# ai4sre/RCAEval

Measured on AMD Instinct MI355X. Metric: Fisher-z CI tests/sec + PC skeleton wall-time (2000 vars), 1/2/4/8 MI355X, higher is better.
Workload: dtype f64

## Files before the change

include/pcgpu.h:

```cpp
#ifndef PCGPU_H
#define PCGPU_H

#include <stdint.h>

#ifdef __cplusplus
extern "C" {
#endif

#define PCG_OK 0
#define PCG_ERR_INVALID -1
#define PCG_ERR_OOM -2
#define PCG_ERR_HIP -3
#define PCG_ERR_SINGULAR -4
#define PCG_ERR_DOMAIN -5
#define PCG_ERR_RCCL -6
#define PCG_ERR_OVERFLOW -7
#define PCG_ERR_PEER -8

#define PCG_FLAG_FULL_P 0x1
#define PCG_FLAG_RECORD 0x2
#define PCG_FLAG_EXACT_ALL 0x4

#define PCG_MAX_LEVELS 32
#define PCG_MAX_DEPTH 12
// ... 28 lines not shown
    int32_t s[PCG_MAX_DEPTH];
    double p;
} pcg_record;

#define PCG_ABI_VERSION 4
int pcg_abi_info(int64_t *stats_bytes, int64_t *record_bytes, int32_t *version);

int pcg_create(int device, pcg_handle **out);
int pcg_destroy(pcg_handle *h);
const char *pcg_last_error(pcg_handle *h);
int pcg_set_stream(pcg_handle *h, void *hip_stream);
int pcg_set_capacity(pcg_handle *h, int64_t record_capacity, int64_t deferred_capacity);
int pcg_set_record_sample(pcg_handle *h, int64_t modulus, int64_t residue);

#define PCG_TUNE_SMALL 0
#define PCG_TUNE_SMALL_QCAP 1
#define PCG_TUNE_LDS_DEEP 2
#define PCG_TUNE_LDS_SPILL_MIN 3
#define PCG_TUNE_WAVE_LO 4
#define PCG_TUNE_SCREEN_MASK 5
#define PCG_TUNE_NODE_BLOCKS 6
#define PCG_TUNE_EXPORT_INLINE 7
#define PCG_TUNE_NB 8
#define PCG_TUNE_NBW 9
#define PCG_TUNE_HOST_TRACE 10
#define PCG_TUNE_K1_I8 11
#define PCG_TUNE_K1_CRT 12
#define PCG_TUNE_K1_CRT_MINN 13
#define PCG_TUNE_K1_CRT_BITS 14
#define PCG_TUNE_K1_CRT_KS 15
#define PCG_TUNE_K1_I8_KS 16
#define PCG_TUNE_K1_SUPER_ORDER 17
#define PCG_TUNE_L1Z 18
#define PCG_TUNE_COUNT 19
int pcg_set_tuning(pcg_handle *h, int key, int64_t value);
int pcg_get_tuning(pcg_handle *h, int key, int64_t *value);

int pcg_corr(pcg_handle *h, const double *X, int64_t N, int64_t n, int64_t ldx,
             double *C, int64_t ldc);

int pcg_corr_shard_bytes(pcg_handle *h, int64_t n, int64_t N, int world, int64_t *bytes_per_rank);
int pcg_k1_plan_signature(pcg_handle *h, int64_t n, int64_t N, int64_t *signature);
int pcg_corr_shard_rows(int64_t n, int world, int64_t *rows_per_rank);
int pcg_corr_shard(pcg_handle *h, const double *X, int64_t N, int64_t n, int64_t ldx, int rank,
                   int world, double *packed);
int pcg_corr_shard_finish(pcg_handle *h, const double *gathered, int64_t N, int64_t n, int world,
                          double *C, int64_t ldc);

int pcg_skeleton(pcg_handle *h, const double *C, int64_t n, int64_t ldc, int64_t N,
                 double alpha, int max_depth, int flags, int8_t *removed_level,
                 pcg_stats *stats);

int pcg_pc_skeleton(pcg_handle *h, const double *X, int64_t N, int64_t n, int64_t ldx, double *C,
                    int64_t ldc, double alpha, int max_depth, int flags, int8_t *removed_level,
                    pcg_stats *stats);

int pcg_degrees(pcg_handle *h, int32_t *deg_host, int64_t capacity);

int pcg_sepset_count(pcg_handle *h, int64_t *count, int32_t *words_per_row);
int pcg_sepset_export(pcg_handle *h, int32_t *xy_host ,
                      uint64_t *bits_host , int64_t count);
int pcg_sepset_export_device(pcg_handle *h, int32_t *xy_dev, uint64_t *bits_dev, int64_t count);
int pcg_set_sepset_buffers(pcg_handle *h, int32_t *xy_dev, uint64_t *bits_dev, int64_t capacity);
int pcg_sepset_target(pcg_handle *h, int32_t *in_caller, int64_t *capacity_needed);

int pcg_record_count(pcg_handle *h, int64_t *count, int64_t *near_alpha_count);
int pcg_record_export(pcg_handle *h, pcg_record *rec_host, int64_t count,
                      pcg_record *near_host, int64_t near_count);

typedef struct {
    const double *X;
    int64_t N, n, ldx;
    double *C;
    int64_t ldc;
    int8_t *removed_level;
// ... 111 lines not shown
```

rcaeval_amd/_lib.py:

```python
from __future__ import annotations

import ctypes
import os

_HERE = os.path.dirname(os.path.abspath(__file__))
LIB_PATH = os.environ.get("PCG_LIB_PATH") or os.path.join(_HERE, "libpcgpu.so")

PCG_OK = 0
PCG_ERR_INVALID = -1
PCG_ERR_OOM = -2
PCG_ERR_HIP = -3
PCG_ERR_SINGULAR = -4
PCG_ERR_DOMAIN = -5
PCG_ERR_RCCL = -6
PCG_ERR_OVERFLOW = -7
PCG_ERR_PEER = -8

PCG_FLAG_FULL_P = 0x1
PCG_FLAG_RECORD = 0x2
PCG_FLAG_EXACT_ALL = 0x4

PCG_MAX_LEVELS = 32
PCG_ABI_VERSION = 4
PCG_RM_STATUS = 64
PCG_MAX_DEPTH = 12
PCG_MAX_LEVEL_DEPTH = 30

PCG_DRIVER_LEVELS = 0
PCG_DRIVER_SMALL = 1
PCG_DRIVER_SMALL_RERUN = 2
DRIVER_NAMES = {PCG_DRIVER_LEVELS: "levels", PCG_DRIVER_SMALL: "small", PCG_DRIVER_SMALL_RERUN: "small_rerun"}

TUNE_KEYS = {
    "SMALL": 0, "SMALL_QCAP": 1, "LDS_DEEP": 2, "LDS_SPILL_MIN": 3, "WAVE_LO": 4, "SCREEN_MASK": 5,
    "NODE_BLOCKS": 6, "EXPORT_INLINE": 7, "NB": 8, "NBW": 9, "HOST_TRACE": 10, "K1_I8": 11, "K1_CRT": 12,
    "K1_CRT_MINN": 13, "K1_CRT_BITS": 14, "K1_CRT_KS": 15, "K1_I8_KS": 16, "K1_SUPER_ORDER": 17,
    "L1Z": 18,
}

I64 = ctypes.c_int64
I32 = ctypes.c_int32
P = ctypes.c_void_p
D = ctypes.c_double


class PcgStats(ctypes.Structure):
    _fields_ = [
        ("tests", I64 * PCG_MAX_LEVELS),
        ("calls", I64 * PCG_MAX_LEVELS),
        ("indep", I64 * PCG_MAX_LEVELS),
        ("exact", I64 * PCG_MAX_LEVELS),
        ("near_alpha", I64 * PCG_MAX_LEVELS),
        ("edges_after", I64 * PCG_MAX_LEVELS),
        ("max_degree", I32 * PCG_MAX_LEVELS),
        ("level_ms", D * PCG_MAX_LEVELS),
        ("kernel_ms", D * PCG_MAX_LEVELS),
        ("levels", I32),
        ("error", I32),
        ("screened", I64 * PCG_MAX_LEVELS),
        ("driver", I32),
        ("driver_pad", I32),
    ]

    def as_dict(self) -> dict:
        L = self.levels
        return {
            "levels": L,
            "error": self.error,
            "tests": list(self.tests[:L]),
            "calls": list(self.calls[:L]),
            "indep": list(self.indep[:L]),
# ... 3 lines not shown
            "max_degree": list(self.max_degree[:L]),
            "level_ms": list(self.level_ms[:L]),
            "kernel_ms": list(self.kernel_ms[:L]),
            "screened": list(self.screened[:L]),
            "driver": DRIVER_NAMES.get(self.driver, str(self.driver)),
        }


class PcgRecord(ctypes.Structure):
    _fields_ = [("a", I32), ("b", I32), ("d", I32), ("s", I32 * PCG_MAX_DEPTH), ("p", D)]


class PcgCase(ctypes.Structure):
    _fields_ = [("X", P), ("N", I64), ("n", I64), ("ldx", I64), ("C", P), ("ldc", I64),
                ("removed_level", P), ("sep_xy", P), ("sep_bits", P)]


class PcgCaseResult(ctypes.Structure):
    _fields_ = [("rc", I32), ("rc_pad", I32), ("sep_rows", I64), ("near_alpha_count", I64),
                ("stats", PcgStats), ("deg", (I32 * 64) * PCG_MAX_LEVELS)]


SIGNATURES = [
    ("pcg_abi_info", I32, [ctypes.POINTER(I64), ctypes.POINTER(I64), ctypes.POINTER(I32)]),
    ("pcg_create", I32, [ctypes.c_int, ctypes.POINTER(P)]),
    ("pcg_destroy", I32, [P]),
    ("pcg_last_error", ctypes.c_char_p, [P]),
    ("pcg_set_stream", I32, [P, P]),
    ("pcg_set_capacity", I32, [P, I64, I64]),
    ("pcg_set_record_sample", I32, [P, I64, I64]),
    ("pcg_set_tuning", I32, [P, ctypes.c_int, I64]),
    ("pcg_get_tuning", I32, [P, ctypes.c_int, ctypes.POINTER(I64)]),
    ("pcg_k1_plan_signature", I32, [P, I64, I64, ctypes.POINTER(I64)]),
    ("pcg_corr", I32, [P, P, I64, I64, I64, P, I64]),
    ("pcg_corr_shard_rows", I32, [I64, ctypes.c_int, ctypes.POINTER(I64)]),
    ("pcg_corr_shard_bytes", I32, [P, I64, I64, ctypes.c_int, ctypes.POINTER(I64)]),
    ("pcg_corr_shard", I32, [P, P, I64, I64, I64, ctypes.c_int, ctypes.c_int, P]),
    ("pcg_corr_shard_finish", I32, [P, P, I64, I64, ctypes.c_int, P, I64]),
    ("pcg_skeleton", I32, [P, P, I64, I64, I64, D, ctypes.c_int, ctypes.c_int, P, ctypes.POINTER(PcgStats)]),
    ("pcg_pc_skeleton", I32, [P, P, I64, I64, I64, P, I64, D, ctypes.c_int, ctypes.c_int, P,
                          ctypes.POINTER(PcgStats)]),
    ("pcg_degrees", I32, [P, P, I64]),
    ("pcg_sepset_count", I32, [P, ctypes.POINTER(I64), ctypes.POINTER(I32)]),
    ("pcg_sepset_export", I32, [P, P, P, I64]),
    ("pcg_sepset_export_device", I32, [P, P, P, I64]),
    ("pcg_set_sepset_buffers", I32, [P, P, P, I64]),
    ("pcg_sepset_target", I32, [P, ctypes.POINTER(I32), ctypes.POINTER(I64)]),
    ("pcg_record_count", I32, [P, ctypes.POINTER(I64), ctypes.POINTER(I64)]),
    ("pcg_record_export", I32, [P, P, I64, P, I64]),
    ("pcg_skeleton_batch", I32, [P, ctypes.POINTER(PcgCase), I64, D, ctypes.c_int, ctypes.c_int,
                                 ctypes.POINTER(PcgCaseResult)]),
    ("pcg_batch_abi_info", I32, [ctypes.POINTER(I64), ctypes.POINTER(I64)]),
    ("pcg_batch_near_export", I32, [P, I64, P, I64]),
    ("pcg_skeleton_init", I32, [P, P, I64, I64, I64, D, ctypes.c_int, P]),
    ("pcg_level_begin", I32, [P, ctypes.c_int, ctypes.POINTER(I64), ctypes.POINTER(I32), ctypes.POINTER(P)]),
    ("pcg_level_run", I32, [P, I64, I64]),
    ("pcg_level_end", I32, [P, ctypes.POINTER(PcgStats)]),
    ("pcg_level_image_totals", I32, [P, ctypes.c_int, ctypes.POINTER(I64), ctypes.POINTER(I64)]),
    ("pcg_level_chunk_work", I32, [P, P, I64]),
    ("pcg_level_split", I32, [P, ctypes.c_int, ctypes.c_int, ctypes.POINTER(I64), ctypes.POINTER(I64)]),
    ("pcg_set_removal_buffer", I32, [P, P, I64]),
    ("pcg_level_packed_words", I32, [I64, ctypes.POINTER(I64)]),
    ("pcg_level_pack", I32, [P, P, ctypes.c_int]),
    ("pcg_level_merge", I32, [P, P, ctypes.c_int]),
    ("pcg_set_world_size", I32, [P, ctypes.c_int]),
    ("pcg_set_narrow_degree", I32, [P, ctypes.c_int]),
# ... 102 lines not shown
```

rcaeval_amd/csrc/api.hip:

```cpp
#include <hip/hip_runtime.h>

#include <algorithm>
#include <cerrno>
#include <cstdlib>
#include <cstring>

#include "handle.h"

int pcg_fail(pcg_handle *h, int code, const char *fmt, ...) {
    if (h) {
        char buf[1024];
        va_list ap;
        va_start(ap, fmt);
        vsnprintf(buf, sizeof(buf), fmt, ap);
        va_end(ap);
        h->err = buf;
    }
    return code;
}

bool pcg_ensure(pcg_handle *h, DevBuf &b, size_t bytes) {
    if (bytes == 0) bytes = 16;
    if (b.bytes >= bytes) return true;
    if (b.p) {
// ... 44 lines not shown
}

extern "C" int pcg_batch_abi_info(int64_t *case_bytes, int64_t *result_bytes) {
    if (case_bytes) *case_bytes = (int64_t)sizeof(pcg_case);
    if (result_bytes) *result_bytes = (int64_t)sizeof(pcg_case_result);
    return PCG_OK;
}

namespace {
struct TuneSpec {
    const char *env;
    int64_t dflt, lo, hi;
};
const TuneSpec kTune[PCG_TUNE_COUNT] = {
    {"PCG_SMALL", 1, 0, 1},
    {"PCG_SMALL_QCAP", 1024, 1, 1024},
    {"PCG_LDS_DEEP", 20, 12, 20},
    {"PCG_LDS_SPILL_MIN", 10000000, 0, INT64_MAX},
    {"PCG_WAVE_LO", 0, 0, PCG_MAX_LEVEL_DEPTH + 1},
    {"PCG_SCREEN_MASK", -1, -1, 0x1c},
    {"PCG_NODE_BLOCKS", 0x18, 0, 0x1c},
    {"PCG_EXPORT_INLINE", 16384, 0, INT64_MAX},
    {"PCG_NB", 0, 0, 1 << 24},
    {"PCG_NBW", 512, 1, 1 << 24},
    {"PCG_HOST_TRACE", 0, 0, 1},
    {"PCG_K1_I8", 1, 0, 1},
    {"PCG_K1_CRT", 1, 0, 1},
    {"PCG_K1_CRT_MINN", 256, 1, 1 << 24},
    {"PCG_K1_CRT_BITS", 53, 32, 63},
    {"PCG_K1_CRT_KS", 0, 0, 16},
    {"PCG_K1_I8_KS", 0, 0, 256},
    {"PCG_K1_SUPER_ORDER", 1, 0, 1},
    {"PCG_L1Z", 1, 0, 1},
};
}

void pcg_tuning_defaults(int64_t *tune) {
    for (int k = 0; k < PCG_TUNE_COUNT; ++k) {
        int64_t v = kTune[k].dflt;
        if (const char *e = getenv(kTune[k].env)) {
            char *end = nullptr;
            errno = 0;
            const long long p = strtoll(e, &end, 0);
            if (end == e || *end != '\0' || errno == ERANGE || p < kTune[k].lo || p > kTune[k].hi)
                fprintf(stderr, "pcgpu: ignoring %s=%s (not an integer in [%lld, %lld]); using %lld\n", kTune[k].env, e,
                        (long long)kTune[k].lo, (long long)kTune[k].hi, (long long)kTune[k].dflt);
            else
                v = p;
        }
        tune[k] = v;
    }
}

extern "C" int pcg_set_tuning(pcg_handle *h, int key, int64_t value) {
    if (!h || key < 0 || key >= PCG_TUNE_COUNT || value < kTune[key].lo || value > kTune[key].hi)
        return pcg_fail(h, PCG_ERR_INVALID, "pcg_set_tuning: key %d value %lld", key, (long long)value);
    h->tune[key] = value;
    return PCG_OK;
}

extern "C" int pcg_get_tuning(pcg_handle *h, int key, int64_t *value) {
    if (!h || !value || key < 0 || key >= PCG_TUNE_COUNT)
        return pcg_fail(h, PCG_ERR_INVALID, "pcg_get_tuning: key %d", key);
    *value = h->tune[key];
    return PCG_OK;
}
// ... 99 lines not shown
```

rcaeval_amd/csrc/corr.hip:

```cpp
#include <hip/hip_runtime.h>

#include <algorithm>
#include <cmath>
#include <cstring>
#include <vector>

#include "handle.h"

namespace {

typedef double d4 __attribute__((ext_vector_type(4)));

#ifndef PCG_K1_TILE
#define PCG_K1_TILE 64
#endif
#ifndef PCG_K1_XCD
#define PCG_K1_XCD 1
#endif
#ifndef PCG_K1_KS
#define PCG_K1_KS 0
#endif
constexpr int TILE = PCG_K1_TILE;
constexpr int WT = TILE / 32;
constexpr int RS = 256 / TILE;
// ... 389 lines not shown
}

constexpr int CRT_KMAX = 24;
constexpr int CRT_L = 6;
constexpr int CRT_T = 256;
constexpr int CRT_KB = 4;
#ifndef PCG_CRT_PR
#define PCG_CRT_PR 8
#endif
constexpr int CRT_PR = PCG_CRT_PR;
#ifndef PCG_CRT_KP
#define PCG_CRT_KP 1
#endif
constexpr int CRT_KP = PCG_CRT_KP;
constexpr int CRT_PL = CRT_PR - 2 * CRT_KP;
static_assert(CRT_PR * 16384 <= 160 * 1024 && CRT_PL >= CRT_KP && CRT_PL % CRT_KP == 0, "CRT LDS ring");
constexpr int CRT_MAXKB = 4095;
constexpr int CRT_UNIT = CRT_T * CRT_T;
static const int kCrtModuli[CRT_KMAX] = {256, 255, 253, 251, 247, 241, 239, 233, 229, 227, 223, 217,
                                         211, 199, 197, 193, 191, 181, 179, 173, 167, 163, 157, 151};

struct CrtTab {
    int k, b, L;
    int m[CRT_KMAX];
    int y[CRT_KMAX];
    float finv[CRT_KMAX];
    double dinv[CRT_KMAX];
    uint32_t wlo[CRT_KMAX], whi[CRT_KMAX];
    uint32_t cneg[CRT_KMAX];
    uint32_t Mi[CRT_KMAX][2 * CRT_L];
    uint32_t M[2 * CRT_L];
};

template <int L>
struct CrtAcc {
    uint32_t l[2 * L];
    float fs;
};

template <int L>
__device__ __forceinline__ void crt_acc_init(CrtAcc<L> &a) {
#pragma unroll
    for (int l = 0; l < 2 * L; ++l) a.l[l] = 0;
    a.fs = 0.0f;
}

template <int L>
__device__ __forceinline__ void crt_acc_add(CrtAcc<L> &a, uint32_t z, int mi, const CrtTab &tab) {
    a.fs = fmaf((float)z, tab.finv[mi], a.fs);
#pragma unroll
    for (int l = 0; l < 2 * L; ++l) a.l[l] = __umul24(z, tab.Mi[mi][l]) + a.l[l];
}

template <int L>
__device__ __forceinline__ double crt_value(const CrtAcc<L> &a, const CrtTab &tab, int ei, int ej) {
    const int32_t qq = (int32_t)floorf(a.fs + 0.5f);
    uint32_t lim[CRT_L];
    int32_t carry = 0;
#pragma unroll
    for (int l = 0; l < CRT_L; ++l) {
        int32_t v0 = carry, v1;
        if (l < L) v0 += (int32_t)a.l[2 * l] - qq * (int32_t)tab.M[2 * l];
        const uint32_t lo = (uint32_t)v0 & 0xffffu;
        v1 = v0 >> 16;
        if (l < L) v1 += (int32_t)a.l[2 * l + 1] - qq * (int32_t)tab.M[2 * l + 1];
        lim[l] = lo | ((uint32_t)v1 << 16);
// ... 87 lines not shown
        const int m = tab.m[mi];
        if (m == 256) {
#pragma unroll
            for (int q = 0; q < 4; ++q) pk[q] = (int)pack4(lo[4 * q], lo[4 * q + 1], lo[4 * q + 2], lo[4 * q + 3]);
        } else {
            const f2 fi = {tab.finv[mi], tab.finv[mi]};
            const f2 nm = {-(float)m, -(float)m};
            const f2 mg = {12582912.0f, 12582912.0f};
            const uint32_t wl = tab.wlo[mi], wh = tab.whi[mi], cn = tab.cneg[mi];
#pragma unroll
            for (int q = 0; q < 4; ++q) {
                uint32_t bb[4];
#pragma unroll
                for (int u = 0; u < 4; u += 2) {
                    const int i = 4 * q + u;
                    const float x0 = (float)(int)__builtin_amdgcn_udot4(
                        lo[i], wl, __builtin_amdgcn_udot4(hi[i], wh, cn, false), false);
                    const float x1 = (float)(int)__builtin_amdgcn_udot4(
                        lo[i + 1], wl, __builtin_amdgcn_udot4(hi[i + 1], wh, cn, false), false);
                    const f2 x = {x0, x1};
                    const f2 qv = __builtin_elementwise_fma(x, fi, mg) - mg;
                    const f2 rv = __builtin_elementwise_fma(qv, nm, x) + mg;
                    const float r0 = rv.x, r1 = rv.y;
                    bb[u] = __float_as_uint(r0);
                    bb[u + 1] = __float_as_uint(r1);
                }
                pk[q] = (int)pack4(bb[0], bb[1], bb[2], bb[3]);
            }
        }
        *reinterpret_cast<v4i *>(dst + mi * plane) = pk;
    }
}

__global__ __launch_bounds__(512, 1) void k_xtx_crt(const int8_t *R, int TB, int64_t plane, int T, int ntiles, int ks,
                                                  int kb, CrtTab tab, int64_t u0, int64_t nu, uint8_t *out) {
    extern __shared__ __attribute__((aligned(16))) unsigned char smem[];
    int64_t lin = blockIdx.x;
    {
        const int64_t per = gridDim.x / 8;
        lin = (blockIdx.x % 8) * per + blockIdx.x / 8;
        if (lin >= nu) return;
    }
    const int64_t u = u0 + lin;
    const int t = (int)(u % ntiles);
    const int64_t sm = u / ntiles;
    const int mi = (int)(sm / ks), slab = (int)(sm % ks);
    int bi, bj;
    tile_of(t, T, bi, bj);
    const int tb0 = slab * kb, tb1 = min(TB, tb0 + kb);
    const int tid = threadIdx.x, lane = tid & 63, w = tid >> 6;
    const int r = lane & 31, hh = lane >> 5;
    const int wr = w >> 2, wc = w & 3;

    v16i acc[4][2];
#pragma unroll
    for (int a = 0; a < 4; ++a)
#pragma unroll
        for (int b = 0; b < 2; ++b)
#pragma unroll
            for (int q = 0; q < 16; ++q) acc[a][b][q] = 0;

    const int8_t *Rm = R + (int64_t)mi * plane;
    const int8_t *srcA = Rm + (int64_t)(bi * 4 + (tid >> 7)) * TB * 2048 + (tid & 127) * 16;
    const int8_t *srcB = Rm + (int64_t)(bj * 4 + (tid >> 7)) * TB * 2048 + (tid & 127) * 16;
    const int nkb = tb1 - tb0;
    auto stage = [&](int g) {
        const int64_t tb = tb0 + min(g, nkb - 1);
        unsigned char *dst = smem + (g % CRT_PR) * 16384 + w * 1024;
        __builtin_amdgcn_global_load_lds((const __attribute__((address_space(1))) void *)(srcA + tb * 2048),
                                         (__attribute__((address_space(3))) void *)dst, 16, 0, 0);
        __builtin_amdgcn_global_load_lds((const __attribute__((address_space(1))) void *)(srcB + tb * 2048),
                                         (__attribute__((address_space(3))) void *)(dst + 8192), 16, 0, 0);
    };
    const unsigned char *fa0 = smem + (2 * wr * 2048 + hh * 1024 + r * 16);
    const unsigned char *fb0 = smem + (8192 + wc * 2048 + hh * 1024 + r * 16);
    v4i af[2][CRT_KP][4], bf[2][CRT_KP][2];
    auto frag = [&](int g, int sl) {
#pragma unroll
// ... 51 lines not shown
#pragma unroll
    for (int a = 0; a < 4; ++a)
#pragma unroll
        for (int b = 0; b < 2; ++b) {
            v4i pk = {0, 0, 0, 0};
#pragma unroll
            for (int q = 0; q < 16; ++q) {
                const int v = acc[a][b][q];
                uint32_t rr;
                if (m == 256) {
                    rr = (uint32_t)v & 255u;
                } else {
                    const int t = __mul24(v >> 16, c16) + (v & 0xffff);
                    const float tf = (float)t;
                    int x = (int)fmaf(-rintf(tf * finv), fm, tf);
                    x += x < 0 ? m : 0;
                    x -= x >= m ? m : 0;
                    rr = (uint32_t)x;
                }
                pk[q >> 2] |= (int)(rr << (8 * (q & 3)));
            }
            *reinterpret_cast<v4i *>(o + (a * 2 + b) * 1024) = pk;
        }
}

__device__ __forceinline__ int crt_unit_offset(int li, int lj) {
    const int wr = li >> 7, a = (li >> 5) & 3, rr = li & 31;
    const int hh = (rr >> 2) & 1, q = (rr & 3) | ((rr >> 3) << 2);
    const int wc = lj >> 6, b = (lj >> 5) & 1, r = lj & 31;
    return ((((wr * 4 + wc) * 4 + a) * 2 + b) * 64 + r + 32 * hh) * 16 + q;
}

template <int L>
__global__ __launch_bounds__(256) void k_crt_diag(const uint8_t *Rs, int T, int ntiles, int ks, CrtTab tab,
                                                 const int *expo, int n, double scale, double *sd) {
    const int i = blockIdx.x * blockDim.x + threadIdx.x;
    if (i >= n) return;
    const int bi = i / CRT_T;
    const int t = bi * T - bi * (bi - 1) / 2;
    const int ei = expo[i];
    if (ei == K1_NONFINITE) {
        sd[i] = NAN;
        return;
    }
    const int k = tab.k;
    const int64_t ustride = (int64_t)ntiles * CRT_UNIT;
    const uint8_t *src = Rs + (int64_t)t * CRT_UNIT + crt_unit_offset(i % CRT_T, i % CRT_T);
    uint32_t sv[CRT_KMAX];
#pragma unroll
    for (int mi = 0; mi < CRT_KMAX; ++mi) sv[mi] = 0;
    for (int s = 0; s < ks; ++s) {
        uint32_t b[CRT_KMAX];
#pragma unroll
        for (int mi = 0; mi < CRT_KMAX; ++mi) b[mi] = src[((int64_t)min(mi, k - 1) * ks + s) * ustride];
#pragma unroll
        for (int mi = 0; mi < CRT_KMAX; ++mi) sv[mi] += b[mi];
    }
    CrtAcc<L> acc;
    crt_acc_init(acc);
#pragma unroll
    for (int mi = 0; mi < CRT_KMAX; ++mi)
        if (mi < k) crt_acc_add(acc, crt_mod(__umul24(sv[mi], (uint32_t)tab.y[mi]), tab.m[mi], tab.finv[mi]), mi, tab);
    sd[i] = sqrt(crt_value(acc, tab, ei, ei) * scale);
}

template <int L>
__global__ __launch_bounds__(256) void k_crt_finish(const uint8_t *Rs, int T, int ntiles, int ks, CrtTab tab,
                                                   const int *expo, int n, const double *sd, double scale, double *C,
                                                   int64_t ldc) {
    const int64_t gid = (int64_t)blockIdx.x * blockDim.x + threadIdx.x;
    const int t = (int)(gid >> 14), rem = (int)((gid >> 2) & 4095), g = (int)(gid & 3);
    if (t >= ntiles) return;
    int bi, bj;
    tile_of(t, T, bi, bj);
    const int lane = rem & 63, wab = rem >> 6;
    const int r = lane & 31, hh = lane >> 5;
    const int b = wab & 1, a = (wab >> 1) & 3, wr = wab >> 5, wc = (wab >> 3) & 3;
    const int j = bj * CRT_T + wc * 64 + b * 32 + r;
    const int ibase = bi * CRT_T + wr * 128 + a * 32 + 4 * hh + 8 * g;
    if (j >= n || ibase > j) return;
    const int k = tab.k;
    const int ej = expo[j];
    const int64_t ustride = (int64_t)ntiles * CRT_UNIT;
    const uint8_t *src = Rs + (int64_t)t * CRT_UNIT + rem * 16 + 4 * g;
    uint32_t se[CRT_KMAX], so[CRT_KMAX];
#pragma unroll
    for (int mi = 0; mi < CRT_KMAX; ++mi) se[mi] = so[mi] = 0;
    for (int s = 0; s < ks; ++s) {
        uint32_t wd[CRT_KMAX];
#pragma unroll
        for (int mi = 0; mi < CRT_KMAX; ++mi)
            wd[mi] = *reinterpret_cast<const uint32_t *>(src + ((int64_t)min(mi, k - 1) * ks + s) * ustride);
#pragma unroll
        for (int mi = 0; mi < CRT_KMAX; ++mi) {
            se[mi] += wd[mi] & 0x00ff00ffu;
            so[mi] += (wd[mi] >> 8) & 0x00ff00ffu;
        }
    }
    CrtAcc<L> acc[4];
#pragma unroll
    for (int q4 = 0; q4 < 4; ++q4) crt_acc_init(acc[q4]);
#pragma unroll
    for (int mi = 0; mi < CRT_KMAX; ++mi) {
        if (mi >= k) continue;
        const int m = tab.m[mi];
        const float fi = tab.finv[mi];
        const uint32_t y = (uint32_t)tab.y[mi];
#pragma unroll
        for (int q4 = 0; q4 < 4; ++q4) {
            const uint32_t sv = (((q4 & 1) ? so[mi] : se[mi]) >> (16 * (q4 >> 1))) & 0xffffu;
            crt_acc_add(acc[q4], crt_mod(__umul24(sv, y), m, fi), mi, tab);
        }
    }
    const double sj = sd[j];
#pragma unroll
    for (int q4 = 0; q4 < 4; ++q4) {
        const int i = ibase + q4;
// ... 2 lines not shown
        const double gv = (ei == K1_NONFINITE || ej == K1_NONFINITE) ? NAN : crt_value(acc[q4], tab, ei, ej);
        const double si = sd[i];
        C[(int64_t)i * ldc + j] = corr_of(gv, scale, si, sj);
        if (i != j) C[(int64_t)j * ldc + i] = corr_of(gv, scale, sj, si);
    }
}

int split_k_i8(const int64_t *tune, int n, int64_t N, int *kb_out) {
    const int T = (n + 63) / 64;
    const int ntiles = T * (T + 1) / 2;
    const int TB = (int)((N + 63) / 64 * 2);
    int ks = (int)std::max<int64_t>(1, (PCG_K1_BLOCKS + ntiles / 2) / ntiles);
    if (tune[PCG_TUNE_K1_I8_KS] > 0) ks = (int)tune[PCG_TUNE_K1_I8_KS];
    ks = std::min(ks, std::max(1, TB / 2));
    ks = std::min(ks, 256);
    int kb = (TB + ks - 1) / ks;
    kb = std::min(kb, K1_I8_MAXK / K1_TB);
    *kb_out = kb;
    return (TB + kb - 1) / kb;
}

struct K1Tune {
    int64_t v[PCG_TUNE_COUNT];
    explicit K1Tune(const pcg_handle *h) {
        if (h) memcpy(v, h->tune, sizeof(v));
        else pcg_tuning_defaults(v);
    }
};

struct CrtPlan {
    CrtTab tab;
    int T = 0, ntiles = 0, ks = 0, kb = 0, TB = 0, CBp = 0;
    int64_t units = 0;
};

static void big_mul_small(uint32_t *x, int L, uint32_t m) {
    uint64_t c = 0;
    for (int l = 0; l < L; ++l) {
        const uint64_t v = (uint64_t)x[l] * m + c;
        x[l] = (uint32_t)v;
        c = v >> 32;
    }
}
static uint32_t big_div_small(const uint32_t *x, int L, uint32_t m, uint32_t *q) {
    uint64_t r = 0;
    for (int l = L - 1; l >= 0; --l) {
        const uint64_t v = (r << 32) | x[l];
        q[l] = (uint32_t)(v / m);
        r = v % m;
    }
    return (uint32_t)r;
}

static bool crt_plan_build(const int64_t *tune, int n, int64_t N, CrtPlan &p);

bool crt_plan(const int64_t *tune, int n, int64_t N, CrtPlan &p) {
    struct Entry {
        int64_t key[7];
        bool ok;
        CrtPlan plan;
    };
    thread_local Entry e{{-1, -1, -1, -1, -1, -1, -1}, false, CrtPlan{}};
    const int64_t key[7] = {n, N, tune[PCG_TUNE_K1_I8], tune[PCG_TUNE_K1_CRT], tune[PCG_TUNE_K1_CRT_MINN],
                            tune[PCG_TUNE_K1_CRT_BITS], tune[PCG_TUNE_K1_CRT_KS]};
    if (memcmp(key, e.key, sizeof(key)) != 0) {
        e.ok = crt_plan_build(tune, n, N, e.plan);
        memcpy(e.key, key, sizeof(key));
    }
    if (e.ok) p = e.plan;
    return e.ok;
}

static bool crt_plan_build(const int64_t *tune, int n, int64_t N, CrtPlan &p) {
    if (!tune[PCG_TUNE_K1_I8] || !tune[PCG_TUNE_K1_CRT] || n < tune[PCG_TUNE_K1_CRT_MINN]) return false;
    const int bmin = (int)std::min<int64_t>(63, std::max<int64_t>(32, tune[PCG_TUNE_K1_CRT_BITS]));
    double lm = 0.0;
    int k = 0, b = 0;
    for (; k < CRT_KMAX; ++k) {
        lm += std::log2((double)kCrtModuli[k]);
        b = (int)std::floor((lm - std::log2((double)N) - 1.0 - 0.01) / 2.0);
        if (b >= bmin) { ++k; break; }
    }
    if (b < bmin) return false;
    b = std::min(b, 63);
    CrtTab &t = p.tab;
    memset(&t, 0, sizeof(t));
    t.k = k;
    t.b = b;
    uint32_t M[CRT_L] = {1, 0, 0, 0, 0, 0};
    for (int i = 0; i < k; ++i) big_mul_small(M, CRT_L, (uint32_t)kCrtModuli[i]);
    t.L = (int)std::floor(lm / 32.0) + 1;
    if (lm > 32.0 * t.L - 1.0) ++t.L;
    if (t.L > CRT_L) return false;
    for (int l = 0; l < CRT_L; ++l) {
        t.M[2 * l] = M[l] & 0xffffu;
        t.M[2 * l + 1] = M[l] >> 16;
    }
    for (int i = 0; i < k; ++i) {
        const uint32_t m = (uint32_t)kCrtModuli[i];
        t.m[i] = (int)m;
        t.finv[i] = 1.0f / (float)m;
        t.dinv[i] = 1.0 / (double)m;
        uint32_t Mi32[CRT_L], mq[CRT_L];
        big_div_small(M, CRT_L, m, Mi32);
        for (int l = 0; l < CRT_L; ++l) {
            t.Mi[i][2 * l] = Mi32[l] & 0xffffu;
// ... 15 lines not shown
        t.whi[i] = wh;
        uint64_t pb = 1;
        for (int s2 = 0; s2 < b; ++s2) pb = (pb * 2) % m;
        t.cneg[i] = 0u - (uint32_t)pb;
    }
    p.T = (n + CRT_T - 1) / CRT_T;
    p.ntiles = p.T * (p.T + 1) / 2;
    p.CBp = p.T * 4;
    p.TB = (int)((N + 63) / 64 * 2);
    int best = 1;
    double best_cost = 1e300;
    const int force = (int)tune[PCG_TUNE_K1_CRT_KS];
    for (int ks = 1; ks <= 16; ++ks) {
        int kbk = (p.TB + ks - 1) / ks;
        kbk = (kbk + CRT_KB - 1) / CRT_KB * CRT_KB;
        const int kse = (p.TB + kbk - 1) / kbk;
        if (kse != ks || kbk > CRT_MAXKB) continue;
        const int64_t U = (int64_t)p.ntiles * k * ks;
        const double cost = force > 0 ? (double)std::abs(ks - force)
                                      : (double)((U + 255) / 256) * kbk * 0.3 + (double)U * 0.026;
        if (cost < best_cost) {
            best_cost = cost;
            best = ks;
        }
    }
    {
        int kbk = (p.TB + best - 1) / best;
        kbk = (kbk + CRT_KB - 1) / CRT_KB * CRT_KB;
        if (kbk > CRT_MAXKB) return false;
        p.kb = kbk;
        p.ks = (p.TB + kbk - 1) / kbk;
    }
    p.units = (int64_t)p.ntiles * k * p.ks;
    return true;
}

int crt_residues(pcg_handle *h, const CrtPlan &p, const double *X, int64_t N, int nn, int64_t ldx, const double *mean,
                 const int *expo, int m0, int m1, hipStream_t st, const int8_t **R) {
    const size_t bytes = (size_t)p.tab.k * p.CBp * p.TB * 2048;
    if (!pcg_ensure(h, h->k1_digits, bytes)) return pcg_fail(h, PCG_ERR_OOM, "K1 residue planes (%zu bytes)", bytes);
    hipLaunchKernelGGL(k_residues, dim3((unsigned)p.CBp, (unsigned)(p.TB / 2)), dim3(256), 0, st, X, N, nn, ldx, mean,
                       expo, p.CBp, p.TB, p.tab, m0, m1, (int8_t *)h->k1_digits.p);
    *R = (const int8_t *)h->k1_digits.p;
    return PCG_OK;
}

void crt_gemm(pcg_handle *h, const CrtPlan &p, const int8_t *R, int64_t u0, int64_t nu, uint8_t *out) {
    if (nu <= 0) return;
    const int64_t plane = (int64_t)p.CBp * p.TB * 2048;
    hipLaunchKernelGGL(k_xtx_crt, dim3((unsigned)((nu + 7) / 8 * 8)), dim3(512), CRT_PR * 16384, h->stream, R,
                       p.TB, plane, p.T, p.ntiles, p.ks, p.kb, p.tab, u0, nu, out);
}

void crt_finish(pcg_handle *h, const CrtPlan &p, const uint8_t *Rs, const int *expo, int nn, int64_t N, double *sd,
                double *C, int64_t ldc) {
    const double scale = 1.0 / (double)(N - 1);
    const int64_t threads = (int64_t)p.ntiles * 16384;
#define CRT_LAUNCH(L_)                                                                                       \
    do {                                                                                                     \
        hipLaunchKernelGGL((k_crt_diag<L_>), dim3((unsigned)((nn + 255) / 256)), dim3(256), 0, h->stream, Rs, \
                           p.T, p.ntiles, p.ks, p.tab, expo, nn, scale, sd);                                  \
        hipLaunchKernelGGL((k_crt_finish<L_>), dim3((unsigned)((threads + 255) / 256)), dim3(256), 0,         \
                           h->stream, Rs, p.T, p.ntiles, p.ks, p.tab, expo, nn, (const double *)sd, scale, C, \
                           ldc);                                                                              \
    } while (0)
    if (p.tab.L <= 4) { CRT_LAUNCH(4); }
    else if (p.tab.L == 5) { CRT_LAUNCH(5); }
    else { CRT_LAUNCH(6); }
#undef CRT_LAUNCH
}

int k1_digits(pcg_handle *h, const double *X, int64_t N, int nn, int64_t ldx, const double *mean, const int *expo,
              int *CB, int *TB, const int8_t **Dg) {
    *CB = (nn + 63) / 64;
    *TB = (int)((N + 63) / 64 * 2);
    const size_t bytes = (size_t)K1_DIG * *CB * *TB * 2048;
    if (!pcg_ensure(h, h->k1_digits, bytes)) return pcg_fail(h, PCG_ERR_OOM, "K1 digit planes (%zu bytes)", bytes);
    hipLaunchKernelGGL(k_digits, dim3((unsigned)*CB, (unsigned)(*TB / 2)), dim3(256), 0, h->stream, X, N, nn, ldx,
                       mean, expo, *CB, *TB, (int8_t *)h->k1_digits.p);
    *Dg = (const int8_t *)h->k1_digits.p;
    return PCG_OK;
}

constexpr int NT = 64;
__device__ __forceinline__ double slab_diag_sd(const double *G, int64_t ldg, int64_t slab_stride, int ks, int i,
                                               double scale) {
    double v = 0.0;
    for (int s = 0; s < ks; ++s) v += G[(int64_t)s * slab_stride + (int64_t)i * ldg + i];
    return sqrt(v * scale);
}

__global__ __launch_bounds__(256) void k_normalize_tiles(const double *G, int64_t ldg, int64_t slab_stride, int ks,
                                                         double *C, int64_t ldc, int n, double scale) {
    __shared__ double t[NT][NT + 1];
    __shared__ double sdr[NT], sdc[NT];
    const int T = (n + NT - 1) / NT;
// ... 120 lines not shown
    if (!pcg_ensure(h, h->colmean, sizeof(double) * (parts + nn) + sizeof(int) * nn))
        return pcg_fail(h, PCG_ERR_OOM, "pcg_corr scratch");
    double *part = (double *)h->colmean.p;
    double *mean = part + parts;
    double *pmax = expo_out ? part + (size_t)nn * nchunks : nullptr;
    double *pmin = expo_out ? pmax + (size_t)nn * nchunks : nullptr;
    hipLaunchKernelGGL(k_colsum_partial, dim3((nn + 255) / 256, nchunks), dim3(256), 0, h->stream, X, N, nn, ldx,
                       part, pmax, pmin);
    int *expo = expo_out ? reinterpret_cast<int *>(mean + nn) : nullptr;
    hipLaunchKernelGGL(k_colstats, dim3((nn + 15) / 16), dim3(256), 0, h->stream, (const double *)part,
                       (const double *)pmax, (const double *)pmin, nchunks, nn, N, mean, expo);
    if (expo_out) *expo_out = expo;
    *mean_out = mean;
    return PCG_OK;
}

}

int64_t k1_plan_signature(const pcg_handle *h, int64_t n, int64_t N) {
    const K1Tune t(h);
    CrtPlan cp;
    if (crt_plan(t.v, (int)n, N, cp))
        return ((int64_t)1 << 62) | ((int64_t)cp.tab.k << 48) | ((int64_t)cp.tab.b << 40) | ((int64_t)cp.ks << 32) |
               (cp.units & 0xffffffffll);
    if (!t.v[PCG_TUNE_K1_I8]) return 2;
    int kb = 0;
    const int ks = split_k_i8(t.v, (int)n, N, &kb);
    return ((int64_t)1 << 61) | ((int64_t)ks << 32) | ((int64_t)kb << 8) | (t.v[PCG_TUNE_K1_SUPER_ORDER] ? 1 : 0);
}

extern "C" int pcg_k1_plan_signature(pcg_handle *h, int64_t n, int64_t N, int64_t *signature) {
    if (n < 1 || N < 2 || n > (1 << 24) || !signature) return pcg_fail(h, PCG_ERR_INVALID, "pcg_k1_plan_signature");
    *signature = k1_plan_signature(h, n, N);
    return PCG_OK;
}

extern "C" int pcg_corr_shard_rows(int64_t n, int world, int64_t *rows_per_rank) {
    if (n < 1 || world < 1 || !rows_per_rank) return PCG_ERR_INVALID;
    const int64_t T = (n + TILE - 1) / TILE;
    *rows_per_rank = (int64_t)TILE * 2 * ((T + 2 * world - 1) / (2 * world));
    return PCG_OK;
}

extern "C" int pcg_corr_shard_bytes(pcg_handle *h, int64_t n, int64_t N, int world, int64_t *bytes_per_rank) {
    if (n < 1 || N < 2 || world < 1 || n > (1 << 24) || !bytes_per_rank) return PCG_ERR_INVALID;
    const K1Tune t(h);
    CrtPlan cp;
    if (crt_plan(t.v, (int)n, N, cp)) {
        *bytes_per_rank = (cp.units + world - 1) / world * (int64_t)CRT_UNIT;
        return PCG_OK;
    }
    int64_t rows = 0;
    pcg_corr_shard_rows(n, world, &rows);
    *bytes_per_rank = rows * n * (int64_t)sizeof(double);
    return PCG_OK;
}

static int *colmean_expo(pcg_handle *h, int64_t N, int nn) {
    const int nchunks = (int)((N + MEAN_ROWS - 1) / MEAN_ROWS);
    return reinterpret_cast<int *>((double *)h->colmean.p + (size_t)nn * nchunks * 3 + nn);
}

extern "C" int pcg_corr_shard(pcg_handle *h, const double *X, int64_t N, int64_t n, int64_t ldx, int rank,
                              int world, double *packed) {
    if (!h || !X || !packed || N < 2 || n < 1 || ldx < n || n > (1 << 24) || world < 1 || rank < 0 ||
        rank >= world)
// ... 139 lines not shown
    h->k1_stamp_ok = true;
    const int64_t per = (cp.units + world - 1) / world, u0 = per * rank;
    const int64_t nu = std::max<int64_t>(std::min<int64_t>(per, cp.units - u0), 0);
    if (nu > 0) {
        const int64_t um = (int64_t)cp.ntiles * cp.ks;
        const int m0 = (int)(u0 / um), m1 = (int)((u0 + nu - 1) / um) + 1;
        const int8_t *R = nullptr;
        rc = crt_residues(h, cp, X, N, nn, ldx, mean, expo, m0, m1, h->stream, &R);
        if (rc) return rc;
        crt_gemm(h, cp, R, u0, nu, (uint8_t *)packed);
    }
    PCG_HIP(h, hipGetLastError());
    return PCG_OK;
}

int corr_shard_crt_finish_enqueue(pcg_handle *h, const double *gathered, int64_t N, int64_t n, double *C,
                                  int64_t ldc) {
    const int nn = (int)n;
    CrtPlan cp;
    if (!crt_plan(h->tune, nn, N, cp) || !h->k1_stamp_ok)
        return pcg_fail(h, PCG_ERR_INVALID, "sharded K1 finish: no CRT-mode shard on this handle");
    crt_finish(h, cp, (const uint8_t *)gathered, colmean_expo(h, N, nn), nn, N, (double *)h->pr_scratch.p, C, ldc);
    PCG_HIP(h, hipGetLastError());
    return PCG_OK;
}

int pcg_corr_launch(pcg_handle *h, const double *X, int64_t N, int64_t n, int64_t ldx, double *C, int64_t ldc) {
    if (!h || !X || !C || N < 2 || n < 1 || ldx < n || ldc < n || n > (1 << 24))
        return pcg_fail(h, PCG_ERR_INVALID, "pcg_corr: invalid arguments");
    PCG_HIP(h, hipSetDevice(h->device));
    const int nn = (int)n;
    const double scale = 1.0 / (double)(N - 1);
    CrtPlan cp;
    if (crt_plan(h->tune, nn, N, cp)) {
        double *mean;
        int *expo = nullptr;
        int rc = column_means(h, X, N, nn, ldx, &mean, &expo);
        if (rc) return rc;
        const size_t sbytes = sizeof(double) * (size_t)(nn + 32);
        if (!pcg_ensure(h, h->pr_scratch, sbytes + (size_t)cp.units * CRT_UNIT))
            return pcg_fail(h, PCG_ERR_OOM, "pcg_corr CRT scratch");
        double *sd = (double *)h->pr_scratch.p;
        uint8_t *Rs = (uint8_t *)h->pr_scratch.p + sbytes;
        const int8_t *R = nullptr;
        rc = crt_residues(h, cp, X, N, nn, ldx, mean, expo, 0, cp.tab.k, h->stream, &R);
        if (rc) return rc;
        crt_gemm(h, cp, R, 0, cp.units, Rs);
        crt_finish(h, cp, Rs, expo, nn, N, sd, C, ldc);
        PCG_HIP(h, hipGetLastError());
        return PCG_OK;
    }
    const bool i8 = h->tune[PCG_TUNE_K1_I8] != 0;
    double *mean;
    int *expo = nullptr;
    int rc = column_means(h, X, N, nn, ldx, &mean, i8 ? &expo : nullptr);
    if (rc) return rc;
    const int T = (nn + TILE - 1) / TILE;
    const int ntiles = T * (T + 1) / 2;
    int64_t kchunk = 0;
    int kb = 0;
    const int ks = i8 ? split_k_i8(h->tune, nn, N, &kb) : split_k(nn, N, &kchunk);
    double *G = C;
    int64_t ldg = ldc, stride = 0;
    if (ks > 1) {
        stride = (int64_t)nn * nn;
        if (!pcg_ensure(h, h->pr_scratch, sizeof(double) * (size_t)stride * ks))
            return pcg_fail(h, PCG_ERR_OOM, "pcg_corr split-K slabs");
// ... 150 lines not shown
```

rcaeval_amd/engine.py:

```python
from __future__ import annotations

import contextlib
import ctypes
import time

import numpy as np

from . import _lib
from ._lib import PcgRecord, PcgStats, check

_ENGINES: dict = {}

RECORD_DTYPE = np.dtype([("a", np.int32), ("b", np.int32), ("d", np.int32),
                         ("s", np.int32, _lib.PCG_MAX_DEPTH), ("p", np.float64)], align=True)
assert RECORD_DTYPE.itemsize == ctypes.sizeof(PcgRecord)


def _torch():
    import torch
    return torch


class SkeletonOut:

# ... 74 lines not shown
            self.close()
        except Exception:
            pass

    def get_tuning(self, key: str) -> int:
        v = ctypes.c_int64()
        check(self.h, self.lib.pcg_get_tuning(self.h, _lib.TUNE_KEYS[key], ctypes.byref(v)), "pcg_get_tuning")
        return v.value

    def set_tuning(self, key: str, value: int) -> None:
        check(self.h, self.lib.pcg_set_tuning(self.h, _lib.TUNE_KEYS[key], int(value)), f"pcg_set_tuning({key})")

    @contextlib.contextmanager
    def tuned(self, **knobs):
        old = {k: self.get_tuning(k) for k in knobs}
        try:
            for k, v in knobs.items():
                self.set_tuning(k, v)
            yield self
        finally:
            for k, v in old.items():
                self.set_tuning(k, v)

    def image_totals(self, depth: int) -> tuple:
        hd, dd = ctypes.c_int64(), ctypes.c_int64()
        check(self.h, self.lib.pcg_level_image_totals(self.h, int(depth), ctypes.byref(hd), ctypes.byref(dd)),
              "pcg_level_image_totals")
        return hd.value, dd.value

    def k1_plan_signature(self, n: int, N: int) -> int:
        v = ctypes.c_int64()
        check(self.h, self.lib.pcg_k1_plan_signature(self.h, int(n), int(N), ctypes.byref(v)), "pcg_k1_plan_signature")
        return v.value

    def to_device(self, a) -> "object":
        torch = _torch()
        if isinstance(a, torch.Tensor):
            return a.to(device=self.device, dtype=torch.float64).contiguous()
        arr = np.ascontiguousarray(np.asarray(a, dtype=np.float64))
        return torch.from_numpy(arr).to(self.device)

    def _strided(self, a):
        torch = _torch()
        return (isinstance(a, torch.Tensor) and a.device == self.device and a.dtype == torch.float64
                and a.dim() == 2 and a.shape[1] >= 1 and a.stride(1) == 1 and a.stride(0) >= a.shape[1])

    def _ld(self, a):
        if not self._strided(a):
            a = self.to_device(a)
        if a.dim() != 2:
            raise ValueError("expected a 2-d array")
        return a, (int(a.stride(0)) if a.shape[0] > 1 else int(a.shape[1]))

    def _out_view(self, out, n: int):
        torch = _torch()
        if out is None:
            return torch.empty((n, n), dtype=torch.float64, device=self.device), n
        if not self._strided(out) or tuple(out.shape) != (n, n):
            raise ValueError(f"out= must be a {n} x {n} float64 view on {self.device} with contiguous rows")
        return out, (int(out.stride(0)) if n > 1 else n)

    def sync(self):
        _torch().cuda.synchronize(self.device)

    def corr(self, X, out=None) -> "object":
        Xd, ldx = self._ld(X)
# ... 622 lines not shown
```

Baseline: 1445 billion.

## Split CRT Gram tiles into two K-slab groups chosen by a makespan model

Adds a mixed K-split plan for the CRT int8 correlation GEMM: tiles are divided into two groups with different slab counts. The split is chosen by a cost model that minimises makespan over 32 workers plus a per-byte term, to reduce tail imbalance in the k_xtx_crt grid. The GEMM, diag and finish kernels now index units through the split descriptor, and the diag and finish kernels change how they derive tile indices. A new API exposes the plan. Only the unsharded pcg_corr path uses the mixed plan, and only when the K1_CRT_MIX knob (default 1) is set and K1_CRT_KS is 0.

New measurement: 1465 billion (median of 6 runs). +1.4%, better.

```diff
diff --git a/include/pcgpu.h b/include/pcgpu.h
--- a/include/pcgpu.h
+++ b/include/pcgpu.h
@@ -84,7 +84,11 @@
 #define PCG_TUNE_K1_I8_KS 16
 #define PCG_TUNE_K1_SUPER_ORDER 17
 #define PCG_TUNE_L1Z 18
-#define PCG_TUNE_COUNT 19
+#define PCG_TUNE_K1_CRT_MIX 19
+#define PCG_K1_CRT_MIX_FORCED (1ll << 30)
+#define PCG_K1_CRT_MIX_FORCE(tA, ksA, ksB) \
+    (PCG_K1_CRT_MIX_FORCED | ((int64_t)(tA) << 10) | ((int64_t)(ksA) << 5) | (int64_t)(ksB))
+#define PCG_TUNE_COUNT 20
 int pcg_set_tuning(pcg_handle *h, int key, int64_t value);
 int pcg_get_tuning(pcg_handle *h, int key, int64_t *value);
 
@@ -93,6 +97,7 @@
 
 int pcg_corr_shard_bytes(pcg_handle *h, int64_t n, int64_t N, int world, int64_t *bytes_per_rank);
 int pcg_k1_plan_signature(pcg_handle *h, int64_t n, int64_t N, int64_t *signature);
+int pcg_k1_crt_plan(pcg_handle *h, int64_t n, int64_t N, int64_t *plan);
 int pcg_corr_shard_rows(int64_t n, int world, int64_t *rows_per_rank);
 int pcg_corr_shard(pcg_handle *h, const double *X, int64_t N, int64_t n, int64_t ldx, int rank,
                    int world, double *packed);
diff --git a/rcaeval_amd/_lib.py b/rcaeval_amd/_lib.py
--- a/rcaeval_amd/_lib.py
+++ b/rcaeval_amd/_lib.py
@@ -35,8 +35,12 @@
     "SMALL": 0, "SMALL_QCAP": 1, "LDS_DEEP": 2, "LDS_SPILL_MIN": 3, "WAVE_LO": 4, "SCREEN_MASK": 5,
     "NODE_BLOCKS": 6, "EXPORT_INLINE": 7, "NB": 8, "NBW": 9, "HOST_TRACE": 10, "K1_I8": 11, "K1_CRT": 12,
     "K1_CRT_MINN": 13, "K1_CRT_BITS": 14, "K1_CRT_KS": 15, "K1_I8_KS": 16, "K1_SUPER_ORDER": 17,
-    "L1Z": 18,
+    "L1Z": 18, "K1_CRT_MIX": 19,
 }
+
+
+def k1_crt_mix_force(tA: int, ksA: int, ksB: int) -> int:
+    return (1 << 30) | (int(tA) << 10) | (int(ksA) << 5) | int(ksB)
 
 I64 = ctypes.c_int64
 I32 = ctypes.c_int32
@@ -106,6 +110,7 @@
     ("pcg_set_tuning", I32, [P, ctypes.c_int, I64]),
     ("pcg_get_tuning", I32, [P, ctypes.c_int, ctypes.POINTER(I64)]),
     ("pcg_k1_plan_signature", I32, [P, I64, I64, ctypes.POINTER(I64)]),
+    ("pcg_k1_crt_plan", I32, [P, I64, I64, ctypes.POINTER(I64)]),
     ("pcg_corr", I32, [P, P, I64, I64, I64, P, I64]),
     ("pcg_corr_shard_rows", I32, [I64, ctypes.c_int, ctypes.POINTER(I64)]),
     ("pcg_corr_shard_bytes", I32, [P, I64, I64, ctypes.c_int, ctypes.POINTER(I64)]),
diff --git a/rcaeval_amd/csrc/api.hip b/rcaeval_amd/csrc/api.hip
--- a/rcaeval_amd/csrc/api.hip
+++ b/rcaeval_amd/csrc/api.hip
@@ -100,6 +100,7 @@
     {"PCG_K1_I8_KS", 0, 0, 256},
     {"PCG_K1_SUPER_ORDER", 1, 0, 1},
     {"PCG_L1Z", 1, 0, 1},
+    {"PCG_K1_CRT_MIX", 1, 0, INT32_MAX},
 };
 }
 
diff --git a/rcaeval_amd/csrc/corr.hip b/rcaeval_amd/csrc/corr.hip
--- a/rcaeval_amd/csrc/corr.hip
+++ b/rcaeval_amd/csrc/corr.hip
@@ -445,6 +445,19 @@
     uint32_t M[2 * CRT_L];
 };
 
+struct CrtSplit {
+    int tA, ksA, kbA, ksB, kbB;
+    int64_t nA;
+};
+
+__device__ __forceinline__ void crt_tile_units(const CrtSplit &sp, int ntiles, int t, int &ks, int64_t &base,
+                                               int64_t &ustride) {
+    const bool inA = t < sp.tA;
+    ks = inA ? sp.ksA : sp.ksB;
+    base = inA ? (int64_t)t : sp.nA + (t - sp.tA);
+    ustride = (int64_t)(inA ? sp.tA : ntiles - sp.tA) * CRT_UNIT;
+}
+
 template <int L>
 struct CrtAcc {
     uint32_t l[2 * L];
@@ -598,18 +611,26 @@
     }
 }
 
-__global__ __launch_bounds__(512, 1) void k_xtx_crt(const int8_t *R, int TB, int64_t plane, int T, int ntiles, int ks,
-                                                  int kb, CrtTab tab, int64_t u0, int64_t nu, uint8_t *out) {
+__global__ __launch_bounds__(512, 1) void k_xtx_crt(const int8_t *R, int TB, int64_t plane, int T, int ntiles,
+                                                  CrtSplit sp, CrtTab tab, int64_t u0, int64_t nu, int64_t nuA,
+                                                  unsigned gA, uint8_t *out) {
     extern __shared__ __attribute__((aligned(16))) unsigned char smem[];
-    int64_t lin = blockIdx.x;
+    int64_t lin;
     {
-        const int64_t per = gridDim.x / 8;
-        lin = (blockIdx.x % 8) * per + blockIdx.x / 8;
-        if (lin >= nu) return;
+        const bool blkA = blockIdx.x < gA;
+        const unsigned b = blkA ? blockIdx.x : blockIdx.x - gA;
+        const int64_t per = (blkA ? gA : gridDim.x - gA) / 8;
+        lin = (b % 8) * per + b / 8;
+        if (lin >= (blkA ? nuA : nu - nuA)) return;
+        if (!blkA) lin += nuA;
     }
     const int64_t u = u0 + lin;
-    const int t = (int)(u % ntiles);
-    const int64_t sm = u / ntiles;
+    const bool inA = u < sp.nA;
+    const int64_t v = inA ? u : u - sp.nA;
+    const int tc = inA ? sp.tA : ntiles - sp.tA;
+    const int ks = inA ? sp.ksA : sp.ksB, kb = inA ? sp.kbA : sp.kbB;
+    const int t = (int)(v % tc) + (inA ? 0 : sp.tA);
+    const int64_t sm = v / tc;
     const int mi = (int)(sm / ks), slab = (int)(sm % ks);
     int bi, bj;
     tile_of(t, T, bi, bj);
@@ -727,11 +748,11 @@
 }
 
 template <int L>
-__global__ __launch_bounds__(256) void k_crt_diag(const uint8_t *Rs, int T, int ntiles, int ks, CrtTab tab,
+__global__ __launch_bounds__(256) void k_crt_diag(const uint8_t *Rs, int T, int ntiles, CrtSplit sp, CrtTab tab,
                                                  const int *expo, int n, double scale, double *sd) {
     const int i = blockIdx.x * blockDim.x + threadIdx.x;
     if (i >= n) return;
-    const int bi = i / CRT_T;
+    const int bi = blockIdx.x;
     const int t = bi * T - bi * (bi - 1) / 2;
     const int ei = expo[i];
     if (ei == K1_NONFINITE) {
@@ -739,8 +760,10 @@
         return;
     }
     const int k = tab.k;
-    const int64_t ustride = (int64_t)ntiles * CRT_UNIT;
-    const uint8_t *src = Rs + (int64_t)t * CRT_UNIT + crt_unit_offset(i % CRT_T, i % CRT_T);
+    int ks;
+    int64_t ubase, ustride;
+    crt_tile_units(sp, ntiles, t, ks, ubase, ustride);
+    const uint8_t *src = Rs + ubase * CRT_UNIT + crt_unit_offset(i % CRT_T, i % CRT_T);
     uint32_t sv[CRT_KMAX];
 #pragma unroll
     for (int mi = 0; mi < CRT_KMAX; ++mi) sv[mi] = 0;
@@ -760,11 +783,12 @@
 }
 
 template <int L>
-__global__ __launch_bounds__(256) void k_crt_finish(const uint8_t *Rs, int T, int ntiles, int ks, CrtTab tab,
+__global__ __launch_bounds__(256) void k_crt_finish(const uint8_t *Rs, int T, int ntiles, CrtSplit sp, CrtTab tab,
                                                    const int *expo, int n, const double *sd, double scale, double *C,
                                                    int64_t ldc) {
     const int64_t gid = (int64_t)blockIdx.x * blockDim.x + threadIdx.x;
-    const int t = (int)(gid >> 14), rem = (int)((gid >> 2) & 4095), g = (int)(gid & 3);
+    const int rem = (int)((gid >> 2) & 4095), g = (int)(gid & 3);
+    const int t = (int)(blockIdx.x >> 6);
     if (t >= ntiles) return;
     int bi, bj;
     tile_of(t, T, bi, bj);
@@ -776,8 +800,10 @@
     if (j >= n || ibase > j) return;
     const int k = tab.k;
     const int ej = expo[j];
-    const int64_t ustride = (int64_t)ntiles * CRT_UNIT;
-    const uint8_t *src = Rs + (int64_t)t * CRT_UNIT + rem * 16 + 4 * g;
+    int ks;
+    int64_t ubase, ustride;
+    crt_tile_units(sp, ntiles, t, ks, ubase, ustride);
+    const uint8_t *src = Rs + ubase * CRT_UNIT + rem * 16 + 4 * g;
     uint32_t se[CRT_KMAX], so[CRT_KMAX];
 #pragma unroll
     for (int mi = 0; mi < CRT_KMAX; ++mi) se[mi] = so[mi] = 0;
@@ -846,6 +872,7 @@
     CrtTab tab;
     int T = 0, ntiles = 0, ks = 0, kb = 0, TB = 0, CBp = 0;
     int64_t units = 0;
+    CrtSplit sp{};
 };
 
 static void big_mul_small(uint32_t *x, int L, uint32_t m) {
@@ -866,26 +893,113 @@
     return (uint32_t)r;
 }
 
-static bool crt_plan_build(const int64_t *tune, int n, int64_t N, CrtPlan &p);
-
-bool crt_plan(const int64_t *tune, int n, int64_t N, CrtPlan &p) {
+static bool crt_plan_build(const int64_t *tune, int n, int64_t N, bool mixed, CrtPlan &p);
+
+bool crt_plan(const int64_t *tune, int n, int64_t N, CrtPlan &p, bool mixed = false) {
     struct Entry {
-        int64_t key[7];
+        int64_t key[8];
         bool ok;
         CrtPlan plan;
     };
-    thread_local Entry e{{-1, -1, -1, -1, -1, -1, -1}, false, CrtPlan{}};
-    const int64_t key[7] = {n, N, tune[PCG_TUNE_K1_I8], tune[PCG_TUNE_K1_CRT], tune[PCG_TUNE_K1_CRT_MINN],
-                            tune[PCG_TUNE_K1_CRT_BITS], tune[PCG_TUNE_K1_CRT_KS]};
+    thread_local Entry cache[2] = {{{-1, -1, -1, -1, -1, -1, -1, -1}, false, CrtPlan{}},
+                                   {{-1, -1, -1, -1, -1, -1, -1, -1}, false, CrtPlan{}}};
+    mixed = mixed && tune[PCG_TUNE_K1_CRT_KS] == 0 && tune[PCG_TUNE_K1_CRT_MIX] != 0;
+    Entry &e = cache[mixed ? 1 : 0];
+    const int64_t key[8] = {n, N, tune[PCG_TUNE_K1_I8], tune[PCG_TUNE_K1_CRT], tune[PCG_TUNE_K1_CRT_MINN],
+                            tune[PCG_TUNE_K1_CRT_BITS], tune[PCG_TUNE_K1_CRT_KS],
+                            mixed ? tune[PCG_TUNE_K1_CRT_MIX] : 0};
     if (memcmp(key, e.key, sizeof(key)) != 0) {
-        e.ok = crt_plan_build(tune, n, N, e.plan);
+        e.ok = crt_plan_build(tune, n, N, mixed, e.plan);
         memcpy(e.key, key, sizeof(key));
     }
     if (e.ok) p = e.plan;
     return e.ok;
 }
 
-static bool crt_plan_build(const int64_t *tune, int n, int64_t N, CrtPlan &p) {
+static double crt_makespan(int64_t nA, double la, int64_t nB, double lb, int P) {
+    if (nA == 0) return (double)((nB + P - 1) / P) * lb;
+    const int64_t rA = nA / P, qA = nA % P;
+    const double t0 = (double)rA * la, t1 = t0 + la, tl = qA ? t1 : t0;
+    if (nB == 0) return tl;
+    auto room = [&](double T) {
+        int64_t c = (P - qA) * (int64_t)std::floor((T - t0) / lb + 1e-9);
+        if (qA && T >= t1) c += qA * (int64_t)std::floor((T - t1) / lb + 1e-9);
+        return c;
+    };
+    double best = 1e300;
+    for (int f = 0; f < (qA ? 2 : 1); ++f) {
+        const double base = f ? t1 : t0;
+        int64_t lo = 0, hi = nB;
+        while (lo < hi) {
+            const int64_t mid = (lo + hi) / 2;
+            if (room(base + (double)mid * lb) >= nB) hi = mid;
+            else lo = mid + 1;
+        }
+        best = std::min(best, base + (double)lo * lb);
+    }
+    return std::max(best, tl);
+}
+
+static int crt_slabs(int TB, int want, int *kb) {
+    int best = 0, bd = INT32_MAX;
+    for (int ks = 1; ks <= 16; ++ks) {
+        int kbk = (TB + ks - 1) / ks;
+        kbk = (kbk + CRT_KB - 1) / CRT_KB * CRT_KB;
+        if ((TB + kbk - 1) / kbk != ks || kbk > CRT_MAXKB) continue;
+        if (std::abs(ks - want) < bd) {
+            bd = std::abs(ks - want);
+            best = ks;
+            *kb = kbk;
+        }
+    }
+    return best;
+}
+
+static void crt_plan_mix(int64_t knob, CrtPlan &p) {
+    const int k = p.tab.k, nt = p.ntiles;
+    auto set = [&](int tA, int ksA, int kbA, int ksB, int kbB) {
+        if (tA == 0) { tA = nt; ksA = ksB; kbA = kbB; }
+        if (tA == nt) { ksB = ksA; kbB = kbA; }
+        p.sp = CrtSplit{tA, ksA, kbA, ksB, kbB, (int64_t)k * ksA * tA};
+        p.units = p.sp.nA + (int64_t)k * ksB * (nt - tA);
+        p.ks = ksA;
+        p.kb = kbA;
+    };
+    if (knob & PCG_K1_CRT_MIX_FORCED) {
+        int kbA = 0, kbB = 0;
+        const int tA = (int)std::min<int64_t>((knob >> 10) & 0xfffff, nt);
+        const int ksA = crt_slabs(p.TB, (int)((knob >> 5) & 31), &kbA), ksB = crt_slabs(p.TB, (int)(knob & 31), &kbB);
+        if (ksA && ksB) set(tA, ksA, kbA, ksB, kbB);
+        return;
+    }
+    constexpr double US_KB = 0.41, US_UNIT = 12.6, US_BYTES = 0.026;
+    int ksv[16], kbv[16], nk = 0;
+    for (int ks = 1; ks <= 16; ++ks) {
+        int kb = 0;
+        if (crt_slabs(p.TB, ks, &kb) == ks) { ksv[nk] = ks; kbv[nk++] = kb; }
+    }
+    auto cost = [&](int tA, int a, int b) {
+        const int64_t nA = (int64_t)k * ksv[a] * tA, nB = (int64_t)k * ksv[b] * (nt - tA);
+        return crt_makespan((nA + 7) / 8, kbv[a] * US_KB + US_UNIT, (nB + 7) / 8, kbv[b] * US_KB + US_UNIT, 32) +
+               (double)(nA + nB) * US_BYTES;
+    };
+    double best = 1e300;
+    int bt = nt, ba = 0, bb = 0;
+    for (int a = 0; a < nk; ++a) {
+        const double c = cost(nt, a, a);
+        if (c < best) { best = c; ba = bb = a; }
+    }
+    const int step = std::max(1, nt / 256);
+    for (int tA = step; tA < nt; tA += step)
+        for (int a = 0; a < nk; ++a)
+            for (int b = a + 1; b < nk; ++b) {
+                const double c = cost(tA, a, b);
+                if (c < best) { best = c; bt = tA; ba = a; bb = b; }
+            }
+    if (nk) set(bt, ksv[ba], kbv[ba], ksv[bb], kbv[bb]);
+}
+
+static bool crt_plan_build(const int64_t *tune, int n, int64_t N, bool mixed, CrtPlan &p) {
     if (!tune[PCG_TUNE_K1_I8] || !tune[PCG_TUNE_K1_CRT] || n < tune[PCG_TUNE_K1_CRT_MINN]) return false;
     const int bmin = (int)std::min<int64_t>(63, std::max<int64_t>(32, tune[PCG_TUNE_K1_CRT_BITS]));
     double lm = 0.0;
@@ -967,6 +1081,8 @@
         p.ks = (p.TB + kbk - 1) / kbk;
     }
     p.units = (int64_t)p.ntiles * k * p.ks;
+    p.sp = CrtSplit{p.ntiles, p.ks, p.kb, p.ks, p.kb, p.units};
+    if (mixed) crt_plan_mix(tune[PCG_TUNE_K1_CRT_MIX], p);
     return true;
 }
 
@@ -983,8 +1099,10 @@
 void crt_gemm(pcg_handle *h, const CrtPlan &p, const int8_t *R, int64_t u0, int64_t nu, uint8_t *out) {
     if (nu <= 0) return;
     const int64_t plane = (int64_t)p.CBp * p.TB * 2048;
-    hipLaunchKernelGGL(k_xtx_crt, dim3((unsigned)((nu + 7) / 8 * 8)), dim3(512), CRT_PR * 16384, h->stream, R,
-                       p.TB, plane, p.T, p.ntiles, p.ks, p.kb, p.tab, u0, nu, out);
+    const int64_t nuA = std::min(nu, std::max<int64_t>(p.sp.nA - u0, 0));
+    const unsigned gA = (unsigned)((nuA + 7) / 8 * 8), gB = (unsigned)((nu - nuA + 7) / 8 * 8);
+    hipLaunchKernelGGL(k_xtx_crt, dim3(gA + gB), dim3(512), CRT_PR * 16384, h->stream, R, p.TB, plane, p.T,
+                       p.ntiles, p.sp, p.tab, u0, nu, nuA, gA, out);
 }
 
 void crt_finish(pcg_handle *h, const CrtPlan &p, const uint8_t *Rs, const int *expo, int nn, int64_t N, double *sd,
@@ -993,10 +1111,10 @@
     const int64_t threads = (int64_t)p.ntiles * 16384;
 #define CRT_LAUNCH(L_)                                                                                       \
     do {                                                                                                     \
-        hipLaunchKernelGGL((k_crt_diag<L_>), dim3((unsigned)((nn + 255) / 256)), dim3(256), 0, h->stream, Rs, \
-                           p.T, p.ntiles, p.ks, p.tab, expo, nn, scale, sd);                                  \
+        hipLaunchKernelGGL((k_crt_diag<L_>), dim3((unsigned)((nn + CRT_T - 1) / CRT_T)), dim3(CRT_T), 0,      \
+                           h->stream, Rs, p.T, p.ntiles, p.sp, p.tab, expo, nn, scale, sd);                   \
         hipLaunchKernelGGL((k_crt_finish<L_>), dim3((unsigned)((threads + 255) / 256)), dim3(256), 0,         \
-                           h->stream, Rs, p.T, p.ntiles, p.ks, p.tab, expo, nn, (const double *)sd, scale, C, \
+                           h->stream, Rs, p.T, p.ntiles, p.sp, p.tab, expo, nn, (const double *)sd, scale, C, \
                            ldc);                                                                              \
     } while (0)
     if (p.tab.L <= 4) { CRT_LAUNCH(4); }
@@ -1183,6 +1301,18 @@
 extern "C" int pcg_k1_plan_signature(pcg_handle *h, int64_t n, int64_t N, int64_t *signature) {
     if (n < 1 || N < 2 || n > (1 << 24) || !signature) return pcg_fail(h, PCG_ERR_INVALID, "pcg_k1_plan_signature");
     *signature = k1_plan_signature(h, n, N);
+    return PCG_OK;
+}
+
+extern "C" int pcg_k1_crt_plan(pcg_handle *h, int64_t n, int64_t N, int64_t *plan) {
+    if (n < 1 || N < 2 || n > (1 << 24) || !plan) return pcg_fail(h, PCG_ERR_INVALID, "pcg_k1_crt_plan");
+    const K1Tune t(h);
+    CrtPlan cp;
+    memset(plan, 0, 8 * sizeof(int64_t));
+    if (crt_plan(t.v, (int)n, N, cp, true)) {
+        const int64_t v[8] = {cp.ntiles, cp.tab.k, cp.sp.tA, cp.sp.ksA, cp.sp.kbA, cp.sp.ksB, cp.sp.kbB, cp.units};
+        memcpy(plan, v, sizeof(v));
+    }
     return PCG_OK;
 }
 
@@ -1388,7 +1518,7 @@
     const int nn = (int)n;
     const double scale = 1.0 / (double)(N - 1);
     CrtPlan cp;
-    if (crt_plan(h->tune, nn, N, cp)) {
+    if (crt_plan(h->tune, nn, N, cp, true)) {
         double *mean;
         int *expo = nullptr;
         int rc = column_means(h, X, N, nn, ldx, &mean, &expo);
diff --git a/rcaeval_amd/engine.py b/rcaeval_amd/engine.py
--- a/rcaeval_amd/engine.py
+++ b/rcaeval_amd/engine.py
@@ -130,6 +130,11 @@
         v = ctypes.c_int64()
         check(self.h, self.lib.pcg_k1_plan_signature(self.h, int(n), int(N), ctypes.byref(v)), "pcg_k1_plan_signature")
         return v.value
+
+    def k1_crt_plan(self, n: int, N: int) -> dict:
+        v = (ctypes.c_int64 * 8)()
+        check(self.h, self.lib.pcg_k1_crt_plan(self.h, int(n), int(N), v), "pcg_k1_crt_plan")
+        return dict(zip(("tiles", "moduli", "tA", "ksA", "kbA", "ksB", "kbB", "units"), (int(x) for x in v)))
 
     def to_device(self, a) -> "object":
         torch = _torch()
```
